# fircarpediem/LSS2_Multimodal_nu

Hardware: AMD Instinct MI355X
Metric: BEV frames/sec (6-cam 352x128 -> 200x200x64), full hot path: CamEncode lift + splat + BevEncode (higher is better)
Workload: dtype bf16; 1 GPU; BASELINE configs[1]: model_BEV_TXT LSS hot path, batch=4/GPU, 6 cams 352x128, D=41, 200x200x64 BEV -> BevEncode -> 200x200x4, trunk (EfficientNet) not included: features are the input; batch_per_gpu=4, global_batch=4, parallelism=dp1 (sample-sharded, no collective), precision=bf16

## Files before the change

### lss2_multimodal_nu_amd/csrc/conv_ring.hip

```cpp
#include <type_traits>

#include "conv_launch.h"
#include "lss_device.h"

namespace {

constexpr int RK_SW = 20, RK_SH = 4;
constexpr int RK_PW = 24, RK_PH = 6;
constexpr int RK_KC = 32;
constexpr int RK_POSB = RK_KC * 2;
constexpr int RK_STRIP_PATCH = RK_PH * RK_PW * RK_POSB;
constexpr int RK_SLAB = 128 * RK_KC * 2;
constexpr int RK_SRC_H = 5, RK_SRC_W = 14;
constexpr int RK_SRC_STRIP = RK_SRC_H * RK_SRC_W * RK_POSB;
constexpr int RK_TH = 2 * RK_SH, RK_TW = 2 * RK_SW;
constexpr int RK_TPW = RK_TW + 2, RK_TPH = RK_TH + 2;
constexpr int RK_TPIECE = (RK_TPH * RK_TPW * 4 + 63) / 64;
constexpr int RK_TSRC_H = 7, RK_TSRC_W = 23;
constexpr int RK_TSRC = RK_TSRC_H * RK_TSRC_W * RK_POSB;
constexpr int RK_TSRC_PIECE = (RK_TSRC_H * RK_TSRC_W * 4 + 63) / 64;

struct RingArgs {
  const unsigned short* x;
  const unsigned short* x2;
  const unsigned char* w;
  const float* scale;
  const float* shift;
  unsigned short* y;
  const float* head_w;
  const float* head_b;
  float* head_out;
  int head_n;
  int B, H, W, Cx, C2, up, Hin, Win, Cin, Cout, relu, wt;
  float ry, rx;
  int SX, SY, nstrips, nblk, nch;
  unsigned long long* stats;
};

__device__ __attribute__((aligned(128))) unsigned char lss_ring_zero_page[128];
__device__ int lss_ring_timeouts;

template <int MODE, bool HEAD, int NSL, bool T22>
struct RingLds {
  static constexpr int RING = 0;
  static constexpr int PATCH = NSL * RK_SLAB;
  static constexpr int PBUF = T22 ? RK_TPIECE * 1024 : 4 * RK_STRIP_PATCH;
  static constexpr int SRC = PATCH + 2 * PBUF;
  static constexpr int HEADX = SRC + (MODE == 1 ? (T22 ? RK_TSRC : 4 * RK_SRC_STRIP) : 0);
  static constexpr int FLAGS = HEADX + (HEAD ? 4 * 80 * 4 * 4 : 0);
  static constexpr int TOTAL = FLAGS + 256;
};
constexpr int F_FULL_W = 0, F_FREE_W = 8, F_FULL_P = 16, F_FREE_P = 18, F_HEAD = 20, F_FULL_S = 24, F_FREE_S = 25;

#define RK_TIMEOUT_COUNTER lss_ring_timeouts
#include "ring_prims.h"

typedef __attribute__((ext_vector_type(2))) __bf16 rk_bf16x2;
__device__ __forceinline__ unsigned int rk_pack_bf2(float lo, float hi) {
  const f32x2 v = {lo, hi};
  return __builtin_bit_cast(unsigned int, __builtin_convertvector(v, rk_bf16x2));
}
__device__ __forceinline__ uint4 rk_blend(const uint4& q00, const uint4& q01, const uint4& q10, const uint4& q11,
                                          float lx, float ly) {
  const float w11 = lx * ly, w10 = ly - w11, w01 = lx - w11, w00 = 1.f - lx - ly + w11;
  const unsigned int* u00 = reinterpret_cast<const unsigned int*>(&q00);
  const unsigned int* u01 = reinterpret_cast<const unsigned int*>(&q01);
  const unsigned int* u10 = reinterpret_cast<const unsigned int*>(&q10);
  const unsigned int* u11 = reinterpret_cast<const unsigned int*>(&q11);
  uint4 out;
  unsigned int* o = reinterpret_cast<unsigned int*>(&out);
#pragma unroll
  for (int i = 0; i < 4; ++i) {
    float lo = __builtin_bit_cast(float, u00[i] << 16) * w00;
    float hi = __builtin_bit_cast(float, u00[i] & 0xffff0000u) * w00;
    lo = __builtin_fmaf(__builtin_bit_cast(float, u01[i] << 16), w01, lo);
    hi = __builtin_fmaf(__builtin_bit_cast(float, u01[i] & 0xffff0000u), w01, hi);
    lo = __builtin_fmaf(__builtin_bit_cast(float, u10[i] << 16), w10, lo);
    hi = __builtin_fmaf(__builtin_bit_cast(float, u10[i] & 0xffff0000u), w10, hi);
    lo = __builtin_fmaf(__builtin_bit_cast(float, u11[i] << 16), w11, lo);
    hi = __builtin_fmaf(__builtin_bit_cast(float, u11[i] & 0xffff0000u), w11, hi);
    o[i] = rk_pack_bf2(lo, hi);
  }
  return out;
}

#ifndef RK_PSLEEP
#define RK_PSLEEP 8
#endif
#ifndef RK_PRIO_C
#define RK_PRIO_C 0
#endif
#ifndef RK_PRIO_P
#define RK_PRIO_P 3
#endif
#ifndef RK_PRIO_W
#define RK_PRIO_W 2
#endif
constexpr int RK_NS = 4;
constexpr int RK_NCONS = 2 * RK_NS;
constexpr int RK_NPATCH = 3;
constexpr int RK_NWAVES = RK_NCONS + 1 + RK_NPATCH;

struct RingTile {
  int nb;
  int b[RK_NS], oy0[RK_NS], ox0[RK_NS];
  bool ok[RK_NS];
};

template <int MODE, bool HEAD, int NSL, bool T22>
__global__ __launch_bounds__(RK_NWAVES * 64, 3) void conv_ring_kernel(RingArgs a) {
  static_assert(!T22 || MODE == 1, "shared tile: fused upsample only");
  using L = RingLds<MODE, HEAD, NSL, T22>;
  constexpr int PW = T22 ? RK_TPW : RK_PW;
  constexpr int LA = NSL - 2;
  static_assert(NSL >= 3 && NSL <= 8, "ring depth");
  static_assert(L::TOTAL <= 160 * 1024, "LDS of one CU");
  __shared__ __attribute__((aligned(1024))) unsigned char smem[L::TOTAL];
  const int tid = threadIdx.x, lane = tid & 63;
  const int wave = __builtin_amdgcn_readfirstlane(tid >> 6);
  const rk_flag_t flags = (rk_flag_t)((__attribute__((address_space(3))) unsigned char*)smem + L::FLAGS);
  if (tid < 64) flags[tid] = 0;
  __syncthreads();
  int st0 = 0, st1 = 0;
#ifdef RK_STATS
#define RK_ST(x) x
  const unsigned long long t_entry = a.stats ? __builtin_amdgcn_s_memrealtime() : 0ull;
  auto write_stats = [&]() {
    if (a.stats != nullptr && lane == 0) {
      unsigned long long* o = a.stats + ((size_t)blockIdx.x * RK_NWAVES + wave) * 6;
      o[0] = (unsigned long long)st0; o[1] = (unsigned long long)st1;
      o[2] = __builtin_amdgcn_s_memrealtime() - t_entry; o[3] = t_entry;
    }
  };
#else
#define RK_ST(x)
  auto write_stats = [&]() {};
#endif

  RingTile T;
  {
    const int t = lss_xcd_order(blockIdx.x, gridDim.x);
    T.nb = t % a.nblk;
    const int quad = t / a.nblk;
    if (T22) {
      const int tx = a.SX >> 1, per = tx * (a.SY >> 1);
      const int b = quad / per, rem = quad - b * per, ty = rem / tx;
#pragma unroll
      for (int s = 0; s < RK_NS; ++s) {
        T.ok[s] = true;
        T.b[s] = b;
        T.oy0[s] = ty * RK_TH + (s >> 1) * RK_SH;
        T.ox0[s] = (rem - ty * tx) * RK_TW + (s & 1) * RK_SW;
      }
    } else {
#pragma unroll
      for (int s = 0; s < RK_NS; ++s) {
        int sid = RK_NS * quad + s;
        T.ok[s] = sid < a.nstrips;
        sid = min(sid, a.nstrips - 1);
        const int per = a.SX * a.SY;
        T.b[s] = sid / per;
        const int rem = sid - T.b[s] * per;
        const int sy = rem / a.SX;
        T.oy0[s] = sy * RK_SH;
        T.ox0[s] = (rem - sy * a.SX) * RK_SW;
      }
    }
  }
  const int nsteps = a.nch * 9;

  if (wave == RK_NCONS) {
    __builtin_amdgcn_s_setprio(RK_PRIO_W);
    const unsigned char* wsrc = a.w + (size_t)T.nb * a.nch * 9 * RK_SLAB + lane * 16;
    int slot = 0, gen = 1, pslot = 0, pgen = 1, inflight = 0;
    auto publish_oldest = [&]() {
      switch (inflight) {
        case 1: lss_wait_vmcnt<0>(); break;
        case 2: lss_wait_vmcnt<8>(); break;
        case 3: lss_wait_vmcnt<16>(); break;
        case 4: lss_wait_vmcnt<24>(); break;
        case 5: lss_wait_vmcnt<32>(); break;
        case 6: lss_wait_vmcnt<40>(); break;
        default: lss_wait_vmcnt<48>(); break;
      }
      rk_set(flags + F_FULL_W + pslot, pgen, lane);
      if (++pslot == NSL) { pslot = 0; ++pgen; }
      --inflight;
    };
    for (int i = 0; i < nsteps; ++i) {
      if (gen > 1) {
        int spins = 0;
        while (rk_peek(flags + F_FREE_W + slot) < RK_NCONS * (gen - 1)) {
          if (inflight > 0) {
            publish_oldest();
          } else {
            __builtin_amdgcn_s_sleep(1);
            ++st0;
            if (++spins > RK_SPIN_LIMIT) {
              if (lane == 0) atomicAdd(&lss_ring_timeouts, 1);
              break;
            }
          }
        }
        asm volatile("" ::: "memory");
      }
      unsigned char* dst = smem + L::RING + slot * RK_SLAB;
#ifndef RK_DIAG_NOWDMA
#pragma unroll
      for (int k = 0; k < 8; ++k) lss_glds16(wsrc + (size_t)i * RK_SLAB + k * 1024, dst + k * 1024);
#endif
      ++inflight;
      if (inflight > LA) publish_oldest();
      if (++slot == NSL) { slot = 0; ++gen; }
    }
    while (inflight > 0) publish_oldest();
    lss_wait_vmcnt<0>();
    write_stats();
    return;
  }

  if (wave > RK_NCONS) {
    __builtin_amdgcn_s_setprio(RK_PRIO_P);
    const int pw = wave - RK_NCONS - 1;
    constexpr int NIT = (T22 ? RK_TPIECE : RK_NS * 9) / RK_NPATCH;
    static_assert(NIT * RK_NPATCH == (T22 ? RK_TPIECE : RK_NS * 9), "pieces split evenly over the patch loaders");
    const int nskip = MODE == 1 ? a.C2 / RK_KC : a.nch;
    const unsigned short* xfull = MODE == 1 ? a.x2 : a.x;
    const int cfull = MODE == 1 ? a.C2 : a.Cx;
    int poff[NIT];
    int g_off[MODE == 1 ? NIT : 1];
    constexpr int NWD = MODE == 1 && T22 ? NIT : 1, NWP = MODE == 1 && !T22 ? NIT : 1;
    float g_lx[NWD], g_ly[NWD];
    unsigned int g_wp[NWP];
    constexpr int SRCW = T22 ? RK_TSRC_W : RK_SRC_W;
    constexpr int NSRCP = T22 ? RK_TSRC_PIECE : RK_NS * 5;
    constexpr int NSRC = MODE == 1 ? (NSRCP + RK_NPATCH - 1) / RK_NPATCH : 1;
    int src_o[NSRC];
#pragma unroll
    for (int k = 0; k < NIT; ++k) {
      const int it = pw + k * RK_NPATCH;
      const int s = T22 ? 0 : it / 9, pos = T22 ? it * 16 + (lane >> 2) : (it % 9) * 16 + (lane >> 2);
      const int prow = pos / PW, pcol = pos - prow * PW;
      const int piece = (lane & 3) ^ ((prow & 1) << 1);
      const int sb = s == 0 ? T.b[0] : s == 1 ? T.b[1] : s == 2 ? T.b[2] : T.b[3];
      const int soy = s == 0 ? T.oy0[0] : s == 1 ? T.oy0[1] : s == 2 ? T.oy0[2] : T.oy0[3];
      const int sox = s == 0 ? T.ox0[0] : s == 1 ? T.ox0[1] : s == 2 ? T.ox0[2] : T.ox0[3];
      const bool sok = s == 0 ? T.ok[0] : s == 1 ? T.ok[1] : s == 2 ? T.ok[2] : T.ok[3];
      const int iy = soy - 1 + prow, ix = sox - 1 + pcol;
      const bool used = T22 ? pos < RK_TPH * RK_TPW : pcol < RK_SW + 2;
      const bool in = sok && used && iy >= 0 && iy < a.Hin && ix >= 0 && ix < a.Win;
      poff[k] = (in && cfull > 0) ? ((sb * a.Hin + iy) * a.Win + ix) * cfull + piece * 8 : -1;
      if (MODE == 1) {
        g_off[k] = 0;
        unsigned int g_w = 0;
        if (in) {
          const int wy0 = (int)(a.ry * (float)max(soy - 1, 0)), wx0 = (int)(a.rx * (float)max(sox - 1, 0));
          const float sy = a.ry * (float)iy, sx = a.rx * (float)ix;
          const int y0 = (int)sy, x0 = (int)sx;
          const unsigned int wy = (unsigned int)((sy - (float)y0) * 65536.f + 0.5f);
          const unsigned int wx = (unsigned int)((sx - (float)x0) * 65536.f + 0.5f);
          g_w = min(wx, 65535u) | (min(wy, 65535u) << 16);
          const int fl = (x0 < a.W - 1 ? 1 : 0) | (y0 < a.H - 1 ? 2 : 0) | 4;
          g_off[k] = ((((y0 - wy0) * SRCW + (x0 - wx0)) * 4 + piece) * 16) | fl;
        }
        if constexpr (T22) {
          g_lx[k] = (float)(g_w & 0xffff) * (1.f / 65536.f);
          g_ly[k] = (float)(g_w >> 16) * (1.f / 65536.f);
        } else {
          g_wp[k] = g_w;
        }
      }
    }
    if (MODE == 1) {
#pragma unroll
      for (int k = 0; k < NSRC; ++k) {
        const int it = pw + k * RK_NPATCH;
        const int s = T22 ? 0 : min(it / 5, RK_NS - 1), q = (T22 ? it : it % 5) * 64 + lane;
        const int pos = min(q >> 2, (T22 ? RK_TSRC_H : RK_SRC_H) * SRCW - 1), part = q & 3;
        const int sr = pos / SRCW, sc = pos - sr * SRCW;
        const int sb = s == 0 ? T.b[0] : s == 1 ? T.b[1] : s == 2 ? T.b[2] : T.b[3];
        const int soy = s == 0 ? T.oy0[0] : s == 1 ? T.oy0[1] : s == 2 ? T.oy0[2] : T.oy0[3];
        const int sox = s == 0 ? T.ox0[0] : s == 1 ? T.ox0[1] : s == 2 ? T.ox0[2] : T.ox0[3];
        const int wy0 = (int)(a.ry * (float)max(soy - 1, 0)), wx0 = (int)(a.rx * (float)max(sox - 1, 0));
        src_o[k] = ((sb * a.H + min(wy0 + sr, a.H - 1)) * a.W + min(wx0 + sc, a.W - 1)) * a.Cx + part * 8;
      }
    }
    auto issue_full = [&](int c, int buf) {
      unsigned char* dst = smem + L::PATCH + buf * L::PBUF;
#pragma unroll
      for (int k = 0; k < NIT; ++k) {
        const void* src = poff[k] >= 0 ? (const void*)(xfull + poff[k] + c * RK_KC) : (const void*)lss_ring_zero_page;
        lss_glds16(src, dst + (pw + k * RK_NPATCH) * 1024);
      }
    };
    if (MODE == 0) {
      issue_full(0, 0);
      if (a.nch > 1) {
        issue_full(1, 1);
        lss_wait_vmcnt<NIT>();
      } else {
        lss_wait_vmcnt<0>();
      }
      rk_add1(flags + F_FULL_P + 0, lane);
      for (int c = 0; c < a.nch; ++c) {
        if (c + 1 < a.nch) {
          lss_wait_vmcnt<0>();
          rk_add1(flags + F_FULL_P + ((c + 1) & 1), lane);
        }
        if (c + 2 < a.nch) {
          st0 += rk_wait_ge<RK_PSLEEP>(flags + F_FREE_P + (c & 1), RK_NCONS * ((c >> 1) + 1));
          issue_full(c + 2, c & 1);
        }
      }
    } else {
      auto issue_src = [&](int c) {
        const int cx = c * RK_KC - a.C2;
#pragma unroll
        for (int k = 0; k < NSRC; ++k) {
          const int it = pw + k * RK_NPATCH;
          if (T22) {
            if (it < RK_TSRC_PIECE && it * 64 + lane < RK_TSRC_H * RK_TSRC_W * 4)
              lss_glds16(a.x + src_o[k] + cx, smem + L::SRC + it * 1024);
          } else if (it < RK_NS * 5 && (it % 5) * 64 + lane < RK_SRC_H * RK_SRC_W * 4) {
            lss_glds16(a.x + src_o[k] + cx, smem + L::SRC + (it / 5) * RK_SRC_STRIP + (it % 5) * 1024);
          }
        }
      };
      auto prepare = [&](int c) {
        if (c < nskip) {
          st0 += rk_wait_ge<RK_PSLEEP>(flags + F_FREE_P + (c & 1), RK_NCONS * (c >> 1));
          issue_full(c, c & 1);
        } else {
          st1 += rk_wait_ge(flags + F_FREE_S, RK_NPATCH * (c - nskip));
          issue_src(c);
        }
      };
      prepare(0);
      for (int c = 0; c < a.nch; ++c) {
        lss_wait_vmcnt<0>();
        if (c >= nskip) {
          rk_add1(flags + F_FULL_S, lane);
          st1 += rk_wait_ge(flags + F_FULL_S, RK_NPATCH * (c - nskip + 1));
          st0 += rk_wait_ge<RK_PSLEEP>(flags + F_FREE_P + (c & 1), RK_NCONS * (c >> 1));
          unsigned char* dst = smem + L::PATCH + (c & 1) * L::PBUF;
          uint4 qa[4], qb[4];
          auto corners = [&](int k, uint4* q) {
            const int it = pw + k * RK_NPATCH;
            const unsigned char* p00 = smem + L::SRC + (T22 ? 0 : (it / 9) * RK_SRC_STRIP) + (g_off[k] & 0xfff0);
            const int dx = (g_off[k] & 1) ? 4 * 16 : 0, dy = (g_off[k] & 2) ? SRCW * 4 * 16 : 0;
            q[0] = *reinterpret_cast<const uint4*>(p00);
#if defined(RK_DIAG_ONEREAD)
            q[1] = q[0]; q[2] = q[0]; q[3] = q[0];
            asm volatile("" : "+v"(q[1].x), "+v"(q[2].x), "+v"(q[3].x));
#else
            q[1] = *reinterpret_cast<const uint4*>(p00 + dx);
            q[2] = *reinterpret_cast<const uint4*>(p00 + dy);
            q[3] = *reinterpret_cast<const uint4*>(p00 + dy + dx);
#endif
          };
          auto finish = [&](int k, const uint4* q) {
            uint4 v = make_uint4(0, 0, 0, 0);
#ifndef RK_DIAG_NOBLEND
#if defined(RK_DIAG_READSONLY)
            v.x = q[0].x ^ q[1].x ^ q[2].x ^ q[3].x; v.y = q[0].y ^ q[1].y ^ q[2].y ^ q[3].y;
            v.z = q[0].z ^ q[1].z ^ q[2].z ^ q[3].z; v.w = q[0].w ^ q[1].w ^ q[2].w ^ q[3].w;
#else
            if constexpr (T22)
              v = rk_blend(q[0], q[1], q[2], q[3], g_lx[k], g_ly[k]);
            else
              v = rk_blend(q[0], q[1], q[2], q[3], (float)(g_wp[k] & 0xffff) * (1.f / 65536.f),
                           (float)(g_wp[k] >> 16) * (1.f / 65536.f));
#endif
            const bool in = (g_off[k] & 4) != 0;
            v.x = in ? v.x : 0u; v.y = in ? v.y : 0u; v.z = in ? v.z : 0u; v.w = in ? v.w : 0u;
#endif
            *reinterpret_cast<uint4*>(dst + (pw + k * RK_NPATCH) * 1024 + lane * 16) = v;
          };
          corners(0, qa);
#pragma unroll
          for (int k = 0; k < NIT; k += 2) {
            if (k + 1 < NIT) corners(k + 1, qb);
            finish(k, qa);
            if (k + 1 < NIT) {
              if (k + 2 < NIT) corners(k + 2, qa);
              finish(k + 1, qb);
            }
          }
          lss_wait_lgkm0();
          rk_add1(flags + F_FREE_S, lane);
        }
        if (c + 1 < a.nch && c + 1 >= nskip) prepare(c + 1);
        rk_add1(flags + F_FULL_P + (c & 1), lane);
        if (c + 1 < a.nch && c + 1 < nskip) prepare(c + 1);
      }
    }
    lss_wait_vmcnt<0>();
    write_stats();
    return;
  }

  __builtin_amdgcn_s_setprio(RK_PRIO_C);
  const int sidx = wave >> 1, cg = wave & 1;
  const int n = lane & 15, kq = lane >> 4;
  const int my_b = sidx == 0 ? T.b[0] : sidx == 1 ? T.b[1] : sidx == 2 ? T.b[2] : T.b[3];
  const int my_oy0 = sidx == 0 ? T.oy0[0] : sidx == 1 ? T.oy0[1] : sidx == 2 ? T.oy0[2] : T.oy0[3];
  const int my_ox0 = sidx == 0 ? T.ox0[0] : sidx == 1 ? T.ox0[1] : sidx == 2 ? T.ox0[2] : T.ox0[3];
  const bool my_ok = sidx == 0 ? T.ok[0] : sidx == 1 ? T.ok[1] : sidx == 2 ? T.ok[2] : T.ok[3];
  f32x4 acc[5][4];
#pragma unroll
  for (int j = 0; j < 5; ++j)
#pragma unroll
    for (int t = 0; t < 4; ++t) acc[j][t] = (f32x4){0.f, 0.f, 0.f, 0.f};
  bf16x8 fw[4], fp[5];
#define RK_DSR(dst, addr, off) asm volatile("ds_read_b128 %0, %1 offset:%2" : "=v"(dst) : "v"(addr), "n"(off))
  const unsigned int lanepk =
      (unsigned int)(cg * 4096 + lane * 16) |
      ((unsigned int)((((n >> 2) * PW + (n & 3)) * RK_POSB + (kq << 4)) ^ (((n >> 2) & 1) << 5)) << 16);
  const unsigned int flag_base = (unsigned int)(__UINTPTR_TYPE__)flags;
  const int pconst = L::PATCH + (T22 ? ((sidx >> 1) * RK_SH * PW + (sidx & 1) * RK_SW) * RK_POSB : sidx * RK_STRIP_PATCH);
  auto add1 = [&](int word) {
    unsigned long long save;
    asm volatile("s_mov_b64 %0, exec\n\ts_mov_b64 exec, 1\n\tds_add_u32 %1, %2\n\ts_mov_b64 exec, %0"
                 : "=&s"(save)
                 : "v"(flag_base + 4 * word), "v"(1)
                 : "memory");
  };

  RK_ST(const unsigned long long tc_loop = __builtin_amdgcn_s_memtime(); const unsigned long long tr_loop = __builtin_amdgcn_s_memrealtime();)
  int slot = 0, gen = 1, buf = 0, pgen = 1;
  rk_wait_ge(flags + F_FULL_P + 0, RK_NPATCH);
  rk_wait_ge(flags + F_FULL_W + 0, 1);
  int fnext;
  {
    const int wa = (int)(lanepk & 0xffffu) + L::RING, pa = (int)(lanepk >> 16) + pconst;
    RK_DSR(fw[0], wa, 0);
    RK_DSR(fw[1], wa, 1024);
    asm volatile("ds_read_b32 %0, %1" : "=v"(fnext) : "v"(flag_base + 4 * (F_FULL_W + (1 % NSL))));
    RK_DSR(fp[0], pa, 0 * 4 * RK_POSB);
    RK_DSR(fp[1], pa, 1 * 4 * RK_POSB);
    RK_DSR(fp[2], pa, 2 * 4 * RK_POSB);
    RK_DSR(fp[3], pa, 3 * 4 * RK_POSB);
    RK_DSR(fp[4], pa, 4 * 4 * RK_POSB);
  }

  auto step = [&](auto TAPc, bool last) {
    constexpr int TAP = decltype(TAPc)::value;
    constexpr int NT = (TAP + 1) % 9;
    constexpr int POFF = (NT / 3) * (PW * RK_POSB) + (NT % 3) * RK_POSB;
    {
      const int wa = (int)(lanepk & 0xffffu) + (L::RING + slot * RK_SLAB);
      RK_DSR(fw[2], wa, 2048);
      RK_DSR(fw[3], wa, 3072);
    }
    __builtin_amdgcn_sched_barrier(0);
    asm volatile("s_waitcnt lgkmcnt(6)" : "+v"(fw[0]), "+v"(fw[1]), "+v"(fp[0]));
    acc[0][0] = __builtin_amdgcn_mfma_f32_16x16x32_bf16(fw[0], fp[0], acc[0][0], 0, 0, 0);
    acc[0][1] = __builtin_amdgcn_mfma_f32_16x16x32_bf16(fw[1], fp[0], acc[0][1], 0, 0, 0);
    __builtin_amdgcn_sched_barrier(0);
    int nslot = slot + 1, ngen = gen;
    if (nslot == NSL) { nslot = 0; ++ngen; }
    int nbuf = buf, npgen = pgen;
    if (TAP == 8) {
      nbuf = buf ^ 1;
      if (nbuf == 0) ++npgen;
    }
    const int wan = (int)(lanepk & 0xffffu) + (L::RING + nslot * RK_SLAB);
    __builtin_amdgcn_sched_barrier(0);
    asm volatile("s_waitcnt lgkmcnt(5)" : "+v"(fp[1]));
    acc[1][0] = __builtin_amdgcn_mfma_f32_16x16x32_bf16(fw[0], fp[1], acc[1][0], 0, 0, 0);
    acc[1][1] = __builtin_amdgcn_mfma_f32_16x16x32_bf16(fw[1], fp[1], acc[1][1], 0, 0, 0);
    __builtin_amdgcn_sched_barrier(0);
    const int pan = (int)((lanepk >> 16) ^ (NT / 3 == 1 ? 32u : 0u)) + (pconst + nbuf * L::PBUF);
    const int n2 = nslot + 1 == NSL ? 0 : nslot + 1;
    const unsigned int fa = flag_base + 4 * (F_FULL_W + n2);
    __builtin_amdgcn_sched_barrier(0);
    asm volatile("s_waitcnt lgkmcnt(4)" : "+v"(fp[2]));
    acc[2][0] = __builtin_amdgcn_mfma_f32_16x16x32_bf16(fw[0], fp[2], acc[2][0], 0, 0, 0);
    acc[2][1] = __builtin_amdgcn_mfma_f32_16x16x32_bf16(fw[1], fp[2], acc[2][1], 0, 0, 0);
    __builtin_amdgcn_sched_barrier(0);
    asm volatile("s_waitcnt lgkmcnt(3)" : "+v"(fp[3]));
    acc[3][0] = __builtin_amdgcn_mfma_f32_16x16x32_bf16(fw[0], fp[3], acc[3][0], 0, 0, 0);
    acc[3][1] = __builtin_amdgcn_mfma_f32_16x16x32_bf16(fw[1], fp[3], acc[3][1], 0, 0, 0);
    __builtin_amdgcn_sched_barrier(0);
    asm volatile("s_waitcnt lgkmcnt(2)" : "+v"(fp[4]));
    acc[4][0] = __builtin_amdgcn_mfma_f32_16x16x32_bf16(fw[0], fp[4], acc[4][0], 0, 0, 0);
    acc[4][1] = __builtin_amdgcn_mfma_f32_16x16x32_bf16(fw[1], fp[4], acc[4][1], 0, 0, 0);
    __builtin_amdgcn_sched_barrier(0);
    if (!last) {
      if (__builtin_amdgcn_readfirstlane(fnext) < ngen) st0 += 1 + rk_wait_ge(flags + F_FULL_W + nslot, ngen);
      if (TAP == 8) st1 += rk_wait_ge(flags + F_FULL_P + nbuf, RK_NPATCH * npgen);
      asm volatile("" ::: "memory");
      RK_DSR(fw[0], wan, 0);
      RK_DSR(fw[1], wan, 1024);
      asm volatile("ds_read_b32 %0, %1" : "=v"(fnext) : "v"(fa));
      __builtin_amdgcn_sched_barrier(0);
      asm volatile("s_waitcnt lgkmcnt(3)" : "+v"(fw[2]), "+v"(fw[3]));
    } else {
      asm volatile("s_waitcnt lgkmcnt(0)" : "+v"(fw[2]), "+v"(fw[3]));
    }
    acc[0][2] = __builtin_amdgcn_mfma_f32_16x16x32_bf16(fw[2], fp[0], acc[0][2], 0, 0, 0);
    acc[0][3] = __builtin_amdgcn_mfma_f32_16x16x32_bf16(fw[3], fp[0], acc[0][3], 0, 0, 0);
    __builtin_amdgcn_sched_barrier(0);
    add1(F_FREE_W + slot);
    if (!last) RK_DSR(fp[0], pan, POFF + 0 * 4 * RK_POSB);
    __builtin_amdgcn_sched_barrier(0);
    acc[1][2] = __builtin_amdgcn_mfma_f32_16x16x32_bf16(fw[2], fp[1], acc[1][2], 0, 0, 0);
    acc[1][3] = __builtin_amdgcn_mfma_f32_16x16x32_bf16(fw[3], fp[1], acc[1][3], 0, 0, 0);
    __builtin_amdgcn_sched_barrier(0);
    if (!last) RK_DSR(fp[1], pan, POFF + 1 * 4 * RK_POSB);
    __builtin_amdgcn_sched_barrier(0);
    acc[2][2] = __builtin_amdgcn_mfma_f32_16x16x32_bf16(fw[2], fp[2], acc[2][2], 0, 0, 0);
    acc[2][3] = __builtin_amdgcn_mfma_f32_16x16x32_bf16(fw[3], fp[2], acc[2][3], 0, 0, 0);
    __builtin_amdgcn_sched_barrier(0);
    if (!last) RK_DSR(fp[2], pan, POFF + 2 * 4 * RK_POSB);
    __builtin_amdgcn_sched_barrier(0);
    acc[3][2] = __builtin_amdgcn_mfma_f32_16x16x32_bf16(fw[2], fp[3], acc[3][2], 0, 0, 0);
    acc[3][3] = __builtin_amdgcn_mfma_f32_16x16x32_bf16(fw[3], fp[3], acc[3][3], 0, 0, 0);
    __builtin_amdgcn_sched_barrier(0);
    if (!last) RK_DSR(fp[3], pan, POFF + 3 * 4 * RK_POSB);
    __builtin_amdgcn_sched_barrier(0);
    acc[4][2] = __builtin_amdgcn_mfma_f32_16x16x32_bf16(fw[2], fp[4], acc[4][2], 0, 0, 0);
    acc[4][3] = __builtin_amdgcn_mfma_f32_16x16x32_bf16(fw[3], fp[4], acc[4][3], 0, 0, 0);
    __builtin_amdgcn_sched_barrier(0);
    if (!last) RK_DSR(fp[4], pan, POFF + 4 * 4 * RK_POSB);
    if (TAP == 8) add1(F_FREE_P + buf);
    __builtin_amdgcn_sched_barrier(0);
    slot = nslot; gen = ngen; buf = nbuf; pgen = npgen;
  };
  for (int c = 0; c < a.nch; ++c) {
    step(std::integral_constant<int, 0>{}, false);
    step(std::integral_constant<int, 1>{}, false);
    step(std::integral_constant<int, 2>{}, false);
    step(std::integral_constant<int, 3>{}, false);
    step(std::integral_constant<int, 4>{}, false);
    step(std::integral_constant<int, 5>{}, false);
    step(std::integral_constant<int, 6>{}, false);
    step(std::integral_constant<int, 7>{}, false);
    step(std::integral_constant<int, 8>{}, c + 1 == a.nch);
  }
#undef RK_DSR
  RK_ST(if (a.stats != nullptr && lane == 0) { unsigned long long* o = a.stats + ((size_t)blockIdx.x * RK_NWAVES + wave) * 6; o[2] = __builtin_amdgcn_s_memrealtime() - t_entry; o[4] = __builtin_amdgcn_s_memtime() - tc_loop; o[5] = __builtin_amdgcn_s_memrealtime() - tr_loop; })

  const int ch0 = T.nb * 128 + cg * 64 + kq * 16;
  {
    float sc[16], sh[16];
#pragma unroll
    for (int v4 = 0; v4 < 4; ++v4) {
      f32x4 s4 = {1.f, 1.f, 1.f, 1.f}, h4 = {0.f, 0.f, 0.f, 0.f};
      if (a.scale) s4 = *reinterpret_cast<const f32x4*>(a.scale + ch0 + v4 * 4);
      if (a.shift) h4 = *reinterpret_cast<const f32x4*>(a.shift + ch0 + v4 * 4);
#pragma unroll
      for (int i = 0; i < 4; ++i) { sc[v4 * 4 + i] = s4[i]; sh[v4 * 4 + i] = h4[i]; }
    }
#pragma unroll
    for (int j = 0; j < 5; ++j)
#pragma unroll
      for (int t = 0; t < 4; ++t)
#pragma unroll
        for (int i = 0; i < 4; ++i) {
          float v = acc[j][t][i] * sc[t * 4 + i] + sh[t * 4 + i];
          acc[j][t][i] = a.relu ? fmaxf(v, 0.f) : v;
        }
  }
  const int oy = my_oy0 + (n >> 2);
  if (!HEAD) {
    const __amdgpu_buffer_rsrc_t yrsrc = __builtin_amdgcn_make_buffer_rsrc(
        a.y, 0, a.wt ? (int)((size_t)a.B * a.Hin * a.Win * a.Cout * 2) : 0, 0x00020000);
    const int chs = T.nb * 128 + cg * 64 + kq * 8;
#pragma unroll
    for (int j = 0; j < 5; ++j) {
      const int ox = my_ox0 + j * 4 + (n & 3);
      u32x4 ox_[2];
#pragma unroll
      for (int d = 0; d < 4; ++d) {
        const unsigned lo = rk_pack_bf2(acc[j][d >> 1][(d & 1) * 2], acc[j][d >> 1][(d & 1) * 2 + 1]);
        const unsigned hi = rk_pack_bf2(acc[j][2 + (d >> 1)][(d & 1) * 2], acc[j][2 + (d >> 1)][(d & 1) * 2 + 1]);
        const u32x2 r = __builtin_amdgcn_permlane16_swap(lo, hi, false, false);
        const u32x2 t = __builtin_amdgcn_permlane32_swap(r[0], r[1], false, false);
        ox_[0][d] = t[0];
        ox_[1][d] = t[1];
      }
      if (!my_ok || oy >= a.Hin || ox >= a.Win) continue;
      const size_t o = (((size_t)my_b * a.Hin + oy) * a.Win + ox) * a.Cout + chs;
#pragma unroll
      for (int hf = 0; hf < 2; ++hf) {
        if (a.wt) __builtin_amdgcn_raw_buffer_store_b128(ox_[hf], yrsrc, (int)((o + hf * 32) * 2), 0, 16);
        else *reinterpret_cast<u32x4*>(a.y + o + hf * 32) = ox_[hf];
      }
    }
  } else {
    float part[5];
#pragma unroll
    for (int j = 0; j < 5; ++j) part[j] = 0.f;
    const int c0 = cg * 64 + kq * 16;
#pragma unroll 1
    for (int k = 0; k < 4; ++k) {
      float hw[16];
#pragma unroll
      for (int v4 = 0; v4 < 4; ++v4) {
        f32x4 w4 = {0.f, 0.f, 0.f, 0.f};
        if (k < a.head_n) w4 = *reinterpret_cast<const f32x4*>(a.head_w + (size_t)k * 128 + c0 + v4 * 4);
#pragma unroll
        for (int i = 0; i < 4; ++i) hw[v4 * 4 + i] = w4[i];
      }
#pragma unroll
      for (int j = 0; j < 5; ++j) {
        float s = 0.f;
#pragma unroll
        for (int t = 0; t < 4; ++t)
#pragma unroll
          for (int i = 0; i < 4; ++i) s = fmaf(acc[j][t][i], hw[t * 4 + i], s);
        s += __shfl_xor(s, 16, 64);
        s += __shfl_xor(s, 32, 64);
        if (kq == k) part[j] = s;
      }
    }
    float* hx = reinterpret_cast<float*>(smem + L::HEADX) + sidx * (80 * 4);
    if (cg == 1) {
#pragma unroll
      for (int j = 0; j < 5; ++j) hx[(j * 16 + n) * 4 + kq] = part[j];
      lss_wait_lgkm0();
      rk_set(flags + F_HEAD + sidx, 1, lane);
    } else {
      rk_wait_ge(flags + F_HEAD + sidx, 1);
      if (kq < a.head_n) {
        const float hb = a.head_b[kq];
#pragma unroll
        for (int j = 0; j < 5; ++j) {
          const int ox = my_ox0 + j * 4 + (n & 3);
          const float v = part[j] + hx[(j * 16 + n) * 4 + kq] + hb;
          if (my_ok && oy < a.Hin && ox < a.Win)
            a.head_out[(((size_t)my_b * a.head_n + kq) * a.Hin + oy) * a.Win + ox] = v;
        }
      }
    }
  }
  RK_ST(if (a.stats != nullptr && lane == 0) {
    unsigned long long* o = a.stats + ((size_t)blockIdx.x * RK_NWAVES + wave) * 6;
    o[0] = (unsigned long long)st0; o[1] = (unsigned long long)st1; o[3] = t_entry;
  })
#undef RK_ST
}

template <bool DGRAD>
__global__ void pack_weights_ring_kernel(const float* __restrict__ w, int Cout, int Cin, unsigned short* __restrict__ out) {
  const size_t n = (size_t)Cout * Cin * 9;
  const int nch = Cin / RK_KC;
  for (size_t e = (size_t)blockIdx.x * 256 + threadIdx.x; e < n; e += (size_t)gridDim.x * 256) {
    const int j = e & 7;
    size_t r = e >> 3;
    const int l = r & 63; r >>= 6;
    const int t = r & 3; r >>= 2;
    const int cg = r & 1; r >>= 1;
    const int tap = r % 9; r /= 9;
    const int chunk = r % nch;
    const int nb = r / nch;
    const int co = nb * 128 + cg * 64 + ((l & 15) >> 2) * 16 + 4 * t + (l & 3);
    const int ci = chunk * RK_KC + (l >> 4) * 8 + j;
    out[e] = lss_f2bf(DGRAD ? w[((size_t)ci * Cout + co) * 9 + (8 - tap)] : w[((size_t)co * Cin + ci) * 9 + tap]);
  }
}

}

extern "C" int lss_conv2d_ring_ok(int B, int H, int W, int Cx, int C2, int up, int Cout, int head_n) {
  if (B <= 0 || H <= 0 || W <= 0 || Cx <= 0 || C2 < 0 || up <= 0 || Cout <= 0 || head_n < 0) return 0;
  if (Cout % 128 != 0 || Cx % 32 != 0 || C2 % 32 != 0) return 0;
  if (head_n > 0 && (Cout != 128 || head_n > 4)) return 0;
  const bool fused = up > 1 || C2 > 0;
  const int Hin = H * up, Win = W * up;
  if (fused) {
    if (up < 2) return 0;
    const float ry = Hin > 1 ? (float)(H - 1) / (float)(Hin - 1) : 0.f, rx = Win > 1 ? (float)(W - 1) / (float)(Win - 1) : 0.f;
    if ((int)(ry * (RK_PH - 1) + 0.999f) + 2 > RK_SRC_H || (int)(rx * (RK_SW + 1) + 0.999f) + 2 > RK_SRC_W) return 0;
  }
  if ((long long)B * Hin * Win * (long long)Cout >= (1LL << 31) / 2) return 0;
  if ((long long)B * H * W * (long long)Cx >= (1LL << 31) || (long long)B * Hin * Win * (long long)(C2 > 0 ? C2 : 1) >= (1LL << 31))
    return 0;
  const long long strips = (long long)B * lss_cdiv(Hin, RK_SH) * lss_cdiv(Win, RK_SW);
  return strips / RK_NS * (Cout / 128) >= 96 ? 1 : 0;
}

extern "C" int lss_conv2d_ring_timeouts(void) {
  int v = -1;
  if (hipMemcpyFromSymbol(&v, HIP_SYMBOL(lss_ring_timeouts), sizeof(int), 0, hipMemcpyDeviceToHost) != hipSuccess) return -1;
  return v;
}

extern "C" size_t lss_conv2d_ring_packed_weight_bytes(int Cout, int Cin) {
  if (Cout <= 0 || Cin <= 0 || Cout % 128 != 0 || Cin % RK_KC != 0) return 0;
  return (size_t)Cout * Cin * 9 * 2;
}

extern "C" int lss_conv2d_pack_weights_ring(const float* w_oihw, int Cout, int Cin, void* w_packed, void* stream) {
  LSS_CHECK_PTR(w_oihw); LSS_CHECK_PTR(w_packed);
  if (lss_conv2d_ring_packed_weight_bytes(Cout, Cin) == 0) return LSS_E_SHAPE;
  const size_t n = (size_t)Cout * Cin * 9;
  const int grid = (int)((n + 255) / 256 > 4096 ? 4096 : (n + 255) / 256);
  hipLaunchKernelGGL(pack_weights_ring_kernel<false>, dim3(grid), dim3(256), 0, lss_stream(stream), w_oihw, Cout, Cin,
                     reinterpret_cast<unsigned short*>(w_packed));
  return lss_launch_status();
}

extern "C" int lss_conv2d_pack_weights_ring_dgrad(const float* w_oihw, int Cout, int Cin, void* w_packed, void* stream) {
  LSS_CHECK_PTR(w_oihw); LSS_CHECK_PTR(w_packed);
  if (lss_conv2d_ring_packed_weight_bytes(Cin, Cout) == 0) return LSS_E_SHAPE;
  const size_t n = (size_t)Cout * Cin * 9;
  const int grid = (int)((n + 255) / 256 > 4096 ? 4096 : (n + 255) / 256);
  hipLaunchKernelGGL(pack_weights_ring_kernel<true>, dim3(grid), dim3(256), 0, lss_stream(stream), w_oihw, Cin, Cout,
                     reinterpret_cast<unsigned short*>(w_packed));
  return lss_launch_status();
}

int lss_conv_ring_launch(const void* x, const void* x2, const void* w_ring, const float* scale, const float* shift,
                         void* y, const float* head_w, const float* head_b, float* head_out, int head_n, int B, int H,
                         int W, int Cx, int C2, int up, int Cout, int relu, int wt, hipStream_t st) {
  if (!lss_conv2d_ring_ok(B, H, W, Cx, C2, up, Cout, head_n)) return LSS_E_SHAPE;
  if (relu != 0 && relu != 1) return LSS_E_LAYOUT;
  RingArgs a;
  a.x = reinterpret_cast<const unsigned short*>(x);
  a.x2 = reinterpret_cast<const unsigned short*>(x2);
  a.w = reinterpret_cast<const unsigned char*>(w_ring);
  a.scale = scale; a.shift = shift;
  a.y = reinterpret_cast<unsigned short*>(y);
  a.head_w = head_w; a.head_b = head_b; a.head_out = head_out; a.head_n = head_n;
  a.B = B; a.H = H; a.W = W; a.Cx = Cx; a.C2 = C2; a.up = up;
  a.Hin = H * up; a.Win = W * up; a.Cin = Cx + C2; a.Cout = Cout; a.relu = relu; a.wt = wt;
  a.ry = a.Hin > 1 ? (float)(H - 1) / (float)(a.Hin - 1) : 0.f;
  a.rx = a.Win > 1 ? (float)(W - 1) / (float)(a.Win - 1) : 0.f;
  a.SX = lss_cdiv(a.Win, RK_SW); a.SY = lss_cdiv(a.Hin, RK_SH);
  a.nstrips = B * a.SX * a.SY;
  a.nblk = Cout / 128;
  a.nch = a.Cin / RK_KC;
  a.stats = lss_env_device_ptr("LSS_RING_STATS");
  const bool fused = up > 1 || C2 > 0;
  const bool t22 = fused && a.Hin % RK_TH == 0 && a.Win % RK_TW == 0 &&
                   (int)(a.ry * (RK_TPH - 1) + 0.999f) + 2 <= RK_TSRC_H && (int)(a.rx * (RK_TPW - 1) + 0.999f) + 2 <= RK_TSRC_W;
  const dim3 g((a.nstrips + RK_NS - 1) / RK_NS * a.nblk), blk(RK_NWAVES * 64);
  if (head_n > 0) {
    if (t22) hipLaunchKernelGGL((conv_ring_kernel<1, true, 7, true>), g, blk, 0, st, a);
    else if (fused) hipLaunchKernelGGL((conv_ring_kernel<1, true, 7, false>), g, blk, 0, st, a);
    else hipLaunchKernelGGL((conv_ring_kernel<0, true, 8, false>), g, blk, 0, st, a);
  } else {
    if (t22) hipLaunchKernelGGL((conv_ring_kernel<1, false, 7, true>), g, blk, 0, st, a);
    else if (fused) hipLaunchKernelGGL((conv_ring_kernel<1, false, 7, false>), g, blk, 0, st, a);
    else hipLaunchKernelGGL((conv_ring_kernel<0, false, 8, false>), g, blk, 0, st, a);
  }
  return lss_launch_status();
}
```

Baseline: 12190 frames/s.

## Add wide consumer-wave variant computing all 128 output channels per wave

Adds a WIDE template mode in which each consumer wave covers a whole strip's 128 output channels, instead of two waves splitting it into 64-channel halves. Each patch fragment read from LDS then feeds twice as many MFMAs. The block drops from 12 to 8 waves, and the head reduction no longer needs the LDS exchange between wave pairs. The cost is double the accumulator registers per wave and a lower occupancy bound (2 blocks per CU instead of 3). Most launch paths now use WIDE; the head-fused t22 path keeps the narrow variant.

```diff
diff --git a/lss2_multimodal_nu_amd/csrc/conv_ring.hip b/lss2_multimodal_nu_amd/csrc/conv_ring.hip
--- a/lss2_multimodal_nu_amd/csrc/conv_ring.hip
+++ b/lss2_multimodal_nu_amd/csrc/conv_ring.hip
@@ -40,14 +40,14 @@
 __device__ __attribute__((aligned(128))) unsigned char lss_ring_zero_page[128];
 __device__ int lss_ring_timeouts;
 
-template <int MODE, bool HEAD, int NSL, bool T22>
+template <int MODE, bool HEAD, int NSL, bool T22, bool WIDE>
 struct RingLds {
   static constexpr int RING = 0;
   static constexpr int PATCH = NSL * RK_SLAB;
   static constexpr int PBUF = T22 ? RK_TPIECE * 1024 : 4 * RK_STRIP_PATCH;
   static constexpr int SRC = PATCH + 2 * PBUF;
   static constexpr int HEADX = SRC + (MODE == 1 ? (T22 ? RK_TSRC : 4 * RK_SRC_STRIP) : 0);
-  static constexpr int FLAGS = HEADX + (HEAD ? 4 * 80 * 4 * 4 : 0);
+  static constexpr int FLAGS = HEADX + (HEAD && !WIDE ? 4 * 80 * 4 * 4 : 0);
   static constexpr int TOTAL = FLAGS + 256;
 };
 constexpr int F_FULL_W = 0, F_FREE_W = 8, F_FULL_P = 16, F_FREE_P = 18, F_HEAD = 20, F_FULL_S = 24, F_FREE_S = 25;
@@ -97,9 +97,9 @@
 #define RK_PRIO_W 2
 #endif
 constexpr int RK_NS = 4;
-constexpr int RK_NCONS = 2 * RK_NS;
 constexpr int RK_NPATCH = 3;
-constexpr int RK_NWAVES = RK_NCONS + 1 + RK_NPATCH;
+constexpr int rk_ncons(bool wide) { return wide ? RK_NS : 2 * RK_NS; }
+constexpr int rk_nwaves(bool wide) { return rk_ncons(wide) + 1 + RK_NPATCH; }
 
 struct RingTile {
   int nb;
@@ -107,10 +107,11 @@
   bool ok[RK_NS];
 };
 
-template <int MODE, bool HEAD, int NSL, bool T22>
-__global__ __launch_bounds__(RK_NWAVES * 64, 3) void conv_ring_kernel(RingArgs a) {
+template <int MODE, bool HEAD, int NSL, bool T22, bool WIDE>
+__global__ __launch_bounds__(rk_nwaves(WIDE) * 64, WIDE ? 2 : 3) void conv_ring_kernel(RingArgs a) {
   static_assert(!T22 || MODE == 1, "shared tile: fused upsample only");
-  using L = RingLds<MODE, HEAD, NSL, T22>;
+  using L = RingLds<MODE, HEAD, NSL, T22, WIDE>;
+  constexpr int RK_NCONS = rk_ncons(WIDE), RK_NWAVES = rk_nwaves(WIDE);
   constexpr int PW = T22 ? RK_TPW : RK_PW;
   constexpr int LA = NSL - 2;
   static_assert(NSL >= 3 && NSL <= 8, "ring depth");
@@ -400,17 +401,18 @@
   }
 
   __builtin_amdgcn_s_setprio(RK_PRIO_C);
-  const int sidx = wave >> 1, cg = wave & 1;
+  const int sidx = WIDE ? wave : wave >> 1, cg = WIDE ? 0 : wave & 1;
+  constexpr int NH = WIDE ? 2 : 1;
   const int n = lane & 15, kq = lane >> 4;
   const int my_b = sidx == 0 ? T.b[0] : sidx == 1 ? T.b[1] : sidx == 2 ? T.b[2] : T.b[3];
   const int my_oy0 = sidx == 0 ? T.oy0[0] : sidx == 1 ? T.oy0[1] : sidx == 2 ? T.oy0[2] : T.oy0[3];
   const int my_ox0 = sidx == 0 ? T.ox0[0] : sidx == 1 ? T.ox0[1] : sidx == 2 ? T.ox0[2] : T.ox0[3];
   const bool my_ok = sidx == 0 ? T.ok[0] : sidx == 1 ? T.ok[1] : sidx == 2 ? T.ok[2] : T.ok[3];
-  f32x4 acc[5][4];
+  f32x4 acc[5][4 * NH];
 #pragma unroll
   for (int j = 0; j < 5; ++j)
 #pragma unroll
-    for (int t = 0; t < 4; ++t) acc[j][t] = (f32x4){0.f, 0.f, 0.f, 0.f};
+    for (int t = 0; t < 4 * NH; ++t) acc[j][t] = (f32x4){0.f, 0.f, 0.f, 0.f};
   bf16x8 fw[4], fp[5];
 #define RK_DSR(dst, addr, off) asm volatile("ds_read_b128 %0, %1 offset:%2" : "=v"(dst) : "v"(addr), "n"(off))
   const unsigned int lanepk =
@@ -443,6 +445,7 @@
     RK_DSR(fp[4], pa, 4 * 4 * RK_POSB);
   }
 
+  if constexpr (!WIDE) {
   auto step = [&](auto TAPc, bool last) {
     constexpr int TAP = decltype(TAPc)::value;
     constexpr int NT = (TAP + 1) % 9;
@@ -538,11 +541,115 @@
     step(std::integral_constant<int, 7>{}, false);
     step(std::integral_constant<int, 8>{}, c + 1 == a.nch);
   }
+  } else {
+#define RK_MFMA(a_, w_, p_) asm volatile("v_mfma_f32_16x16x32_bf16 %0, %1, %2, %0" : "+v"(a_) : "v"(w_), "v"(p_))
+#define RK_PAIR(j, t, wA, wB)           \
+  RK_MFMA(acc[j][t], wA, fp[j]);        \
+  RK_MFMA(acc[j][(t) + 1], wB, fp[j]);  \
+  __builtin_amdgcn_sched_barrier(0)
+  auto stepw = [&](auto TAPc, bool last) {
+    constexpr int TAP = decltype(TAPc)::value;
+    constexpr int NT = (TAP + 1) % 9;
+    constexpr int POFF = (NT / 3) * (PW * RK_POSB) + (NT % 3) * RK_POSB;
+    const int wa = (int)(lanepk & 0xffffu) + (L::RING + slot * RK_SLAB);
+    RK_DSR(fw[2], wa, 2 * 1024);
+    RK_DSR(fw[3], wa, 3 * 1024);
+    __builtin_amdgcn_sched_barrier(0);
+    asm volatile("s_waitcnt lgkmcnt(6)" : "+v"(fw[0]), "+v"(fw[1]), "+v"(fp[0]));
+    RK_PAIR(0, 0, fw[0], fw[1]);
+    int nslot = slot + 1, ngen = gen;
+    if (nslot == NSL) { nslot = 0; ++ngen; }
+    int nbuf = buf, npgen = pgen;
+    if (TAP == 8) {
+      nbuf = buf ^ 1;
+      if (nbuf == 0) ++npgen;
+    }
+    const int wan = (int)(lanepk & 0xffffu) + (L::RING + nslot * RK_SLAB);
+    __builtin_amdgcn_sched_barrier(0);
+    asm volatile("s_waitcnt lgkmcnt(5)" : "+v"(fp[1]));
+    RK_PAIR(1, 0, fw[0], fw[1]);
+    const int pan = (int)((lanepk >> 16) ^ (NT / 3 == 1 ? 32u : 0u)) + (pconst + nbuf * L::PBUF);
+    const int n2 = nslot + 1 == NSL ? 0 : nslot + 1;
+    const unsigned int fa = flag_base + 4 * (F_FULL_W + n2);
+    __builtin_amdgcn_sched_barrier(0);
+    asm volatile("s_waitcnt lgkmcnt(4)" : "+v"(fp[2]));
+    RK_PAIR(2, 0, fw[0], fw[1]);
+    asm volatile("s_waitcnt lgkmcnt(3)" : "+v"(fp[3]));
+    RK_PAIR(3, 0, fw[0], fw[1]);
+    asm volatile("s_waitcnt lgkmcnt(2)" : "+v"(fp[4]));
+    RK_PAIR(4, 0, fw[0], fw[1]);
+    RK_DSR(fw[0], wa, 4 * 1024);
+    RK_DSR(fw[1], wa, 5 * 1024);
+    __builtin_amdgcn_sched_barrier(0);
+    asm volatile("s_waitcnt lgkmcnt(2)" : "+v"(fw[2]), "+v"(fw[3]));
+    RK_PAIR(0, 2, fw[2], fw[3]);
+    RK_PAIR(1, 2, fw[2], fw[3]);
+    RK_PAIR(2, 2, fw[2], fw[3]);
+    RK_PAIR(3, 2, fw[2], fw[3]);
+    RK_PAIR(4, 2, fw[2], fw[3]);
+    RK_DSR(fw[2], wa, 6 * 1024);
+    RK_DSR(fw[3], wa, 7 * 1024);
+    __builtin_amdgcn_sched_barrier(0);
+    asm volatile("s_waitcnt lgkmcnt(2)" : "+v"(fw[0]), "+v"(fw[1]));
+    RK_PAIR(0, 4, fw[0], fw[1]);
+    RK_PAIR(1, 4, fw[0], fw[1]);
+    RK_PAIR(2, 4, fw[0], fw[1]);
+    RK_PAIR(3, 4, fw[0], fw[1]);
+    RK_PAIR(4, 4, fw[0], fw[1]);
+    if (!last) {
+      if (__builtin_amdgcn_readfirstlane(fnext) < ngen) st0 += 1 + rk_wait_ge(flags + F_FULL_W + nslot, ngen);
+      if (TAP == 8) st1 += rk_wait_ge(flags + F_FULL_P + nbuf, RK_NPATCH * npgen);
+      asm volatile("" ::: "memory");
+      RK_DSR(fw[0], wan, 0);
+      RK_DSR(fw[1], wan, 1024);
+      asm volatile("ds_read_b32 %0, %1" : "=v"(fnext) : "v"(fa));
+      __builtin_amdgcn_sched_barrier(0);
+      asm volatile("s_waitcnt lgkmcnt(3)" : "+v"(fw[2]), "+v"(fw[3]));
+    } else {
+      asm volatile("s_waitcnt lgkmcnt(0)" : "+v"(fw[2]), "+v"(fw[3]));
+    }
+    RK_PAIR(0, 6, fw[2], fw[3]);
+    add1(F_FREE_W + slot);
+    if (!last) RK_DSR(fp[0], pan, POFF + 0 * 4 * RK_POSB);
+    __builtin_amdgcn_sched_barrier(0);
+    RK_PAIR(1, 6, fw[2], fw[3]);
+    if (!last) RK_DSR(fp[1], pan, POFF + 1 * 4 * RK_POSB);
+    __builtin_amdgcn_sched_barrier(0);
+    RK_PAIR(2, 6, fw[2], fw[3]);
+    if (!last) RK_DSR(fp[2], pan, POFF + 2 * 4 * RK_POSB);
+    __builtin_amdgcn_sched_barrier(0);
+    RK_PAIR(3, 6, fw[2], fw[3]);
+    if (!last) RK_DSR(fp[3], pan, POFF + 3 * 4 * RK_POSB);
+    __builtin_amdgcn_sched_barrier(0);
+    RK_PAIR(4, 6, fw[2], fw[3]);
+    if (!last) RK_DSR(fp[4], pan, POFF + 4 * 4 * RK_POSB);
+    if (TAP == 8) add1(F_FREE_P + buf);
+    __builtin_amdgcn_sched_barrier(0);
+    slot = nslot; gen = ngen; buf = nbuf; pgen = npgen;
+  };
+#undef RK_PAIR
+  for (int c = 0; c < a.nch; ++c) {
+    stepw(std::integral_constant<int, 0>{}, false);
+    stepw(std::integral_constant<int, 1>{}, false);
+    stepw(std::integral_constant<int, 2>{}, false);
+    stepw(std::integral_constant<int, 3>{}, false);
+    stepw(std::integral_constant<int, 4>{}, false);
+    stepw(std::integral_constant<int, 5>{}, false);
+    stepw(std::integral_constant<int, 6>{}, false);
+    stepw(std::integral_constant<int, 7>{}, false);
+    stepw(std::integral_constant<int, 8>{}, c + 1 == a.nch);
+  }
+  asm volatile("s_nop 15\n\ts_nop 15"
+               : "+v"(acc[0][6]), "+v"(acc[0][7]), "+v"(acc[1][6]), "+v"(acc[1][7]), "+v"(acc[2][6]), "+v"(acc[2][7]),
+                 "+v"(acc[3][6]), "+v"(acc[3][7]), "+v"(acc[4][6]), "+v"(acc[4][7]));
+#undef RK_MFMA
+  }
 #undef RK_DSR
   RK_ST(if (a.stats != nullptr && lane == 0) { unsigned long long* o = a.stats + ((size_t)blockIdx.x * RK_NWAVES + wave) * 6; o[2] = __builtin_amdgcn_s_memrealtime() - t_entry; o[4] = __builtin_amdgcn_s_memtime() - tc_loop; o[5] = __builtin_amdgcn_s_memrealtime() - tr_loop; })
 
-  const int ch0 = T.nb * 128 + cg * 64 + kq * 16;
-  {
+#pragma unroll
+  for (int h = 0; h < NH; ++h) {
+    const int ch0 = T.nb * 128 + (cg + h) * 64 + kq * 16;
     float sc[16], sh[16];
 #pragma unroll
     for (int v4 = 0; v4 < 4; ++v4) {
@@ -558,23 +665,26 @@
       for (int t = 0; t < 4; ++t)
 #pragma unroll
         for (int i = 0; i < 4; ++i) {
-          float v = acc[j][t][i] * sc[t * 4 + i] + sh[t * 4 + i];
-          acc[j][t][i] = a.relu ? fmaxf(v, 0.f) : v;
+          float v = acc[j][h * 4 + t][i] * sc[t * 4 + i] + sh[t * 4 + i];
+          acc[j][h * 4 + t][i] = a.relu ? fmaxf(v, 0.f) : v;
         }
   }
   const int oy = my_oy0 + (n >> 2);
   if (!HEAD) {
     const __amdgpu_buffer_rsrc_t yrsrc = __builtin_amdgcn_make_buffer_rsrc(
         a.y, 0, a.wt ? (int)((size_t)a.B * a.Hin * a.Win * a.Cout * 2) : 0, 0x00020000);
-    const int chs = T.nb * 128 + cg * 64 + kq * 8;
+#pragma unroll
+    for (int h = 0; h < NH; ++h) {
+    const int chs = T.nb * 128 + (cg + h) * 64 + kq * 8;
 #pragma unroll
     for (int j = 0; j < 5; ++j) {
       const int ox = my_ox0 + j * 4 + (n & 3);
       u32x4 ox_[2];
 #pragma unroll
       for (int d = 0; d < 4; ++d) {
-        const unsigned lo = rk_pack_bf2(acc[j][d >> 1][(d & 1) * 2], acc[j][d >> 1][(d & 1) * 2 + 1]);
-        const unsigned hi = rk_pack_bf2(acc[j][2 + (d >> 1)][(d & 1) * 2], acc[j][2 + (d >> 1)][(d & 1) * 2 + 1]);
+        const int t0 = h * 4 + (d >> 1);
+        const unsigned lo = rk_pack_bf2(acc[j][t0][(d & 1) * 2], acc[j][t0][(d & 1) * 2 + 1]);
+        const unsigned hi = rk_pack_bf2(acc[j][t0 + 2][(d & 1) * 2], acc[j][t0 + 2][(d & 1) * 2 + 1]);
         const u32x2 r = __builtin_amdgcn_permlane16_swap(lo, hi, false, false);
         const u32x2 t = __builtin_amdgcn_permlane32_swap(r[0], r[1], false, false);
         ox_[0][d] = t[0];
@@ -588,11 +698,14 @@
         else *reinterpret_cast<u32x4*>(a.y + o + hf * 32) = ox_[hf];
       }
     }
+    }
   } else {
-    float part[5];
-#pragma unroll
-    for (int j = 0; j < 5; ++j) part[j] = 0.f;
-    const int c0 = cg * 64 + kq * 16;
+    float part[NH][5];
+#pragma unroll
+    for (int h = 0; h < NH; ++h) {
+#pragma unroll
+    for (int j = 0; j < 5; ++j) part[h][j] = 0.f;
+    const int c0 = (cg + h) * 64 + kq * 16;
 #pragma unroll 1
     for (int k = 0; k < 4; ++k) {
       float hw[16];
@@ -609,16 +722,29 @@
 #pragma unroll
         for (int t = 0; t < 4; ++t)
 #pragma unroll
-          for (int i = 0; i < 4; ++i) s = fmaf(acc[j][t][i], hw[t * 4 + i], s);
+          for (int i = 0; i < 4; ++i) s = fmaf(acc[j][h * 4 + t][i], hw[t * 4 + i], s);
         s += __shfl_xor(s, 16, 64);
         s += __shfl_xor(s, 32, 64);
-        if (kq == k) part[j] = s;
-      }
-    }
+        if (kq == k) part[h][j] = s;
+      }
+    }
+    }
+    if constexpr (WIDE) {
+      if (kq < a.head_n) {
+        const float hb = a.head_b[kq];
+#pragma unroll
+        for (int j = 0; j < 5; ++j) {
+          const int ox = my_ox0 + j * 4 + (n & 3);
+          const float v = part[0][j] + part[NH - 1][j] + hb;
+          if (my_ok && oy < a.Hin && ox < a.Win)
+            a.head_out[(((size_t)my_b * a.head_n + kq) * a.Hin + oy) * a.Win + ox] = v;
+        }
+      }
+    } else {
     float* hx = reinterpret_cast<float*>(smem + L::HEADX) + sidx * (80 * 4);
     if (cg == 1) {
 #pragma unroll
-      for (int j = 0; j < 5; ++j) hx[(j * 16 + n) * 4 + kq] = part[j];
+      for (int j = 0; j < 5; ++j) hx[(j * 16 + n) * 4 + kq] = part[0][j];
       lss_wait_lgkm0();
       rk_set(flags + F_HEAD + sidx, 1, lane);
     } else {
@@ -628,11 +754,12 @@
 #pragma unroll
         for (int j = 0; j < 5; ++j) {
           const int ox = my_ox0 + j * 4 + (n & 3);
-          const float v = part[j] + hx[(j * 16 + n) * 4 + kq] + hb;
+          const float v = part[0][j] + hx[(j * 16 + n) * 4 + kq] + hb;
           if (my_ok && oy < a.Hin && ox < a.Win)
             a.head_out[(((size_t)my_b * a.head_n + kq) * a.Hin + oy) * a.Win + ox] = v;
         }
       }
+    }
     }
   }
   RK_ST(if (a.stats != nullptr && lane == 0) {
@@ -736,15 +863,15 @@
   const bool fused = up > 1 || C2 > 0;
   const bool t22 = fused && a.Hin % RK_TH == 0 && a.Win % RK_TW == 0 &&
                    (int)(a.ry * (RK_TPH - 1) + 0.999f) + 2 <= RK_TSRC_H && (int)(a.rx * (RK_TPW - 1) + 0.999f) + 2 <= RK_TSRC_W;
-  const dim3 g((a.nstrips + RK_NS - 1) / RK_NS * a.nblk), blk(RK_NWAVES * 64);
+  const dim3 g((a.nstrips + RK_NS - 1) / RK_NS * a.nblk), wide(rk_nwaves(true) * 64), narrow(rk_nwaves(false) * 64);
   if (head_n > 0) {
-    if (t22) hipLaunchKernelGGL((conv_ring_kernel<1, true, 7, true>), g, blk, 0, st, a);
-    else if (fused) hipLaunchKernelGGL((conv_ring_kernel<1, true, 7, false>), g, blk, 0, st, a);
-    else hipLaunchKernelGGL((conv_ring_kernel<0, true, 8, false>), g, blk, 0, st, a);
+    if (t22) hipLaunchKernelGGL((conv_ring_kernel<1, true, 7, true, false>), g, narrow, 0, st, a);
+    else if (fused) hipLaunchKernelGGL((conv_ring_kernel<1, true, 7, false, true>), g, wide, 0, st, a);
+    else hipLaunchKernelGGL((conv_ring_kernel<0, true, 8, false, true>), g, wide, 0, st, a);
   } else {
-    if (t22) hipLaunchKernelGGL((conv_ring_kernel<1, false, 7, true>), g, blk, 0, st, a);
-    else if (fused) hipLaunchKernelGGL((conv_ring_kernel<1, false, 7, false>), g, blk, 0, st, a);
-    else hipLaunchKernelGGL((conv_ring_kernel<0, false, 8, false>), g, blk, 0, st, a);
+    if (t22) hipLaunchKernelGGL((conv_ring_kernel<1, false, 7, true, true>), g, wide, 0, st, a);
+    else if (fused) hipLaunchKernelGGL((conv_ring_kernel<1, false, 7, false, true>), g, wide, 0, st, a);
+    else hipLaunchKernelGGL((conv_ring_kernel<0, false, 8, false, true>), g, wide, 0, st, a);
   }
   return lss_launch_status();
 }
```

After: 12240 frames/s, median of 6. Within noise of the previous version (+0.5%).
